# microsoft/VidTok

Hardware: NVIDIA H100
Metric: frames/sec encode+decode, kl_causal_488 17x256x256 (higher is better)
Workload: dtype bf16

## Files before the change

vidtok_b200/csrc/conv_tc.cu:

```cuda
#include <cuda.h>

#include <cstdio>
#include <cstdlib>
#include <cstring>
#include <mutex>
#include <string>
#include <type_traits>

#include "common.cuh"
#include "kernels.h"
#include "tc_host.h"
#include "tc_ptx.cuh"

namespace vt {

namespace {

thread_local std::string g_tc_err;

struct TcParams {
  int B, To, Ho, Wo, Co, Ti;
  int BW, BH, BT;
  int tilesW, tilesH, tilesT;
  int num_n_tiles, BN;
// ... 2 lines not shown
  int st, pt, ph, pw, to_off;
  int sp;
  int t_mode, cacheT;
  int stages;
  const float* bias;
  int res_mode;
  const bf16* res;
  long long rsB, rsT, rsH, rsW;
  int resT, res_t_mode, res_pool_off;
  const bf16* res_cache;
  float ra, rb;
  void* out;
  long long osB, osT, osH, osW, osC;
  int out_f32;
  int Co_real;
  int w_batched;
  int ln_mode, ln_silu;
  const float* ln_gamma;
  const float* ln_beta;
  void* out2;
  int res_mma;
  int halo, hP, a_stages;
  uint32_t halo_bytes;
  int split, a_lo, b_lo, o_lo;
  float acc_scale;
  int kparts;
  int reg_mode, reg_zc, reg_sample;
  const float* reg_noise;
  float* reg_z;
  int* reg_idx;
  double* reg_kl;
  FsqConst reg_fsq;
  uint32_t misc_off;
};

struct TcMaps {
  CUtensorMap a[4];
  CUtensorMap c;
  CUtensorMap b;
  CUtensorMap r;
  CUtensorMap e;
};

constexpr int kConsumerWarps = 8;
constexpr int kProducerWarp = kConsumerWarps;
constexpr int kThreads = (kConsumerWarps + 4) * 32;
constexpr int kABytes = 128 * 128;
constexpr uint32_t kBarTurn = 3, kBarBias = 5;

__host__ __device__ constexpr bool ping_pong(int BN, bool split) { return !split && (BN == 64 || BN == 128); }

using namespace tcx;

struct TileCoord {
  int b, t0, h0, w0, n0;
};
__device__ __forceinline__ TileCoord decode_tile(const TcParams& p, long long tile) {
  TileCoord c;
  const int nt = (int)(tile % p.num_n_tiles);
  long long m = tile / p.num_n_tiles;
  const int tw = (int)(m % p.tilesW); m /= p.tilesW;
  const int th = (int)(m % p.tilesH); m /= p.tilesH;
  const int tt = (int)(m % p.tilesT);
  c.b = (int)(m / p.tilesT);
  c.t0 = tt * p.BT; c.h0 = th * p.BH; c.w0 = tw * p.BW; c.n0 = nt * p.BN;
  return c;
}
__device__ __forceinline__ bool tap_time(const TcParams& p, const TileCoord& tc, int a, int& tv, bool& from_cache) {
  tv = (tc.t0 + p.to_off) * p.st + a - p.pt;
  from_cache = false;
  if (tv + p.BT <= 0) {
    if (p.t_mode == 0) return false;
    if (p.t_mode == 1) { tv = 0; return true; }
    from_cache = true;
    tv = p.cacheT + tv;
    return true;
  }
  return true;
}
__device__ __forceinline__ int tile_taps(const TcParams& p, const TileCoord& tc) {
  int n = 0;
  for (int a = 0; a < p.kt; ++a) {
    int tv;
    bool from_cache;
    if (tap_time(p, tc, a, tv, from_cache)) ++n;
  }
  return n;
}

__device__ __forceinline__ float quad_sum(float v) {
  v += __shfl_xor_sync(0xffffffffu, v, 1);
  v += __shfl_xor_sync(0xffffffffu, v, 2);
  return v;
}

template <int BN, bool kSplit>
__global__ void __launch_bounds__(kThreads, 1)
conv_tc_kernel(const __grid_constant__ TcMaps maps, const TcParams p) {
  extern __shared__ uint8_t smem_raw[];
  const uint32_t smem_base = (smem_u32(smem_raw) + 1023u) & ~1023u;
  uint8_t* smem_gen = smem_raw + (smem_base - smem_u32(smem_raw));
  const int warp = threadIdx.x >> 5, lane = threadIdx.x & 31;
  const uint32_t a_bytes = kABytes;
  constexpr uint32_t b_bytes = (uint32_t)BN * 128u;
  constexpr uint32_t kPl = kSplit ? 2u : 1u;
  const uint32_t stage_bytes = kPl * (p.halo ? b_bytes : a_bytes + b_bytes);
  const uint32_t win_bytes = kPl * p.halo_bytes;
  const uint32_t ring_base = smem_base + (p.halo ? (uint32_t)p.a_stages * win_bytes : 0u);
  const uint32_t bar_base = ring_base + p.stages * stage_bytes;
  auto full_bar = [&](int s) { return bar_base + 8u * s; };
  auto empty_bar = [&](int s) { return bar_base + 8u * (p.stages + s); };
  auto fullA_bar = [&](int s) { return bar_base + 8u * (2 * p.stages + s); };
  auto emptyA_bar = [&](int s) { return bar_base + 8u * (2 * p.stages + p.a_stages + s); };
  constexpr bool kPingPong = ping_pong(BN, kSplit);
  float* sbias = reinterpret_cast<float*>(smem_gen + p.misc_off);
  float* rowbuf = sbias + 2 * 768;

  if (threadIdx.x == 0) {
    constexpr uint32_t readers = kPingPong ? kConsumerWarps / 2 : kConsumerWarps;
    for (int s = 0; s < p.stages; ++s) {
      mbar_init(full_bar(s), 1);
      mbar_init(empty_bar(s), readers);
    }
    for (int s = 0; s < p.a_stages; ++s) {
      mbar_init(fullA_bar(s), 1);
      mbar_init(emptyA_bar(s), readers);
    }
    asm volatile("fence.mbarrier_init.release.cluster;" ::: "memory");
  }
  __syncthreads();

  const int nsp = p.kh * p.kw;
  const int num_kc = p.num_kc, nstages = p.stages;
  const bool halo = p.halo != 0;
  const int res_steps = p.res_mma ? BN / 64 : 0;

  if (warp >= kProducerWarp) {
    asm volatile("setmaxnreg.dec.sync.aligned.u32 40;" ::: "memory");
    if (warp != kProducerWarp) return;
    const bool el = elect_one();
    if (el) {
      prefetch_tmap(&maps.a[0]);
// ... 366 lines not shown
                  constexpr int zc = decltype(ZC)::value;
                  const long long zb = (long long)tc.b * zc * plane + pos;
#pragma unroll
                  for (int c = 0; c < zc; ++c) {
                    float zv;
                    part += kl_sample_one(f[c], f[zc + c], p.reg_sample ? p.reg_noise[zb + c * plane] : 0.f, p.reg_sample, zv);
                    p.reg_z[zb + c * plane] = zv;
                  }
                };
                if (ok) {
                  if (p.reg_zc == 4) kl_row(std::integral_constant<int, 4>());
                  else if (p.reg_zc == 8) kl_row(std::integral_constant<int, 8>());
                  else kl_row(std::integral_constant<int, 16>());
                }
                double dsum = (double)part;
#pragma unroll
                for (int o = 16; o > 0; o >>= 1) dsum += __shfl_xor_sync(0xffffffffu, dsum, o);
                if (lane == 0) atomicAdd(p.reg_kl, dsum);
              } else if (ok) {
                const long long zb = (long long)tc.b * p.reg_zc * plane + pos;
                float idx = 0.f;
#pragma unroll
                for (int c = 0; c < VT_MAX_FSQ; ++c)
                  if (c < p.reg_zc) p.reg_z[zb + c * plane] = fsq_code(p.reg_fsq, c, f[c], idx);
                if (p.reg_idx) p.reg_idx[(long long)tc.b * plane + pos] = (int)idx;
              }
            }
            asm volatile("bar.sync 2, %0;" ::"n"(kConsumerWarps * 32) : "memory");
          }
        }
        continue;
      }

      auto put = [&](void* optr, int r, int c, float y0, float y1) {
        bf16* o = reinterpret_cast<bf16*>(optr) + ooff[r] + tc.n0 + c;
        if constexpr (kSplit) {
          const uint32_t hw = pack_f16x2(y0, y1);
          *reinterpret_cast<uint32_t*>(o) = hw;
          *reinterpret_cast<uint32_t*>(o + p.o_lo) = pack_f16x2(y0 - f16_lo(hw), y1 - f16_hi(hw));
        } else {
          *reinterpret_cast<uint32_t*>(o) = pack_bf16x2(y0, y1);
        }
      };
      if constexpr (kSplit) {
        if (store_a) {
#pragma unroll
          for (int r = 0; r < 2; ++r)
            if (valid[r])
#pragma unroll
              for (int j = 0; j < BN / 8; ++j) put(p.out, r, 8 * j + cq, acc_h[4 * j + 2 * r], acc_h[4 * j + 2 * r + 1]);
        }
        if (p.ln_mode) {
          void* nout = p.ln_mode == 1 ? p.out : p.out2;
#pragma unroll
          for (int r = 0; r < 2; ++r) {
            float s = 0.f;
#pragma unroll
            for (int j = 0; j < BN / 8; ++j) s += acc_h[4 * j + 2 * r] + acc_h[4 * j + 2 * r + 1];
            const float mean = quad_sum(s) * inv_n;
            float q = 0.f;
#pragma unroll
            for (int j = 0; j < BN / 8; ++j) {
              const float d0 = acc_h[4 * j + 2 * r] - mean, d1 = acc_h[4 * j + 2 * r + 1] - mean;
              q = fmaf(d0, d0, q);
              q = fmaf(d1, d1, q);
            }
// ... 17 lines not shown
          for (int j = 0; j < BN / 8; ++j) {
            const float f0 = acc_h[4 * j + 2 * r], f1 = acc_h[4 * j + 2 * r + 1];
            s += f0 + f1;
            q = fmaf(f0, f0, q);
            q = fmaf(f1, f1, q);
            const uint32_t kp = pack_bf16x2(f0, f1);
            if (store_a && valid[r]) *reinterpret_cast<uint32_t*>(reinterpret_cast<bf16*>(p.out) + ooff[r] + tc.n0 + 8 * j + cq) = kp;
            acc_h[4 * j + 2 * r] = bf16_lo(kp);
            acc_h[4 * j + 2 * r + 1] = bf16_hi(kp);
          }
          if (!p.ln_mode) continue;
          const float mean = quad_sum(s) * inv_n;
          float var = fmaf(-mean, mean, quad_sum(q) * inv_n);
          var = var < 0.f ? 0.f : var;
          const float rstd = rsqrtf(var + 1e-6f);
          const float nmr = -mean * rstd;
          if (!valid[r]) continue;
          void* nout = p.ln_mode == 1 ? p.out : p.out2;
#pragma unroll
          for (int j = 0; j < BN / 8; ++j) {
            const int c = 8 * j + cq;
            float y0 = fmaf(fmaf(acc_h[4 * j + 2 * r], rstd, nmr), gamma_s[c], beta_s[c]);
            float y1 = fmaf(fmaf(acc_h[4 * j + 2 * r + 1], rstd, nmr), gamma_s[c + 1], beta_s[c + 1]);
            if (p.ln_silu) {
              y0 = fmaf(y0, tanh_approx(y0), y0);
              y1 = fmaf(y1, tanh_approx(y1), y1);
            }
            put(nout, r, c, y0, y1);
          }
        }
      }
    }
  }
}

__global__ void fill_identity_kernel(bf16* e, int f16, float value) {
  const int r = blockIdx.x, c = threadIdx.x;
  if (f16) reinterpret_cast<__half*>(e)[r * 256 + c] = __float2half_rn(r == c ? value : 0.0f);
  else e[r * 256 + c] = __float2bfloat16_rn(r == c ? value : 0.0f);
}

bool choose_tile(const ConvP& p, int rows, int& BW, int& BH, int& BT) {
  const bool allow_bt = (p.st == 1) && (p.t_mode == 0);
  long long best = -1;
  auto ceil_to = [](int v, int b) { return (long long)((v + b - 1) / b) * b; };
  for (int bw = 128; bw >= 8; bw >>= 1) {
    for (int bh = rows / bw; bh >= 1; bh >>= 1) {
      if (bh > 256) continue;
      const int bt = rows / (bw * bh);
      if (bt > 1 && !allow_bt) continue;
      if (bt > 16) continue;
      const long long padded = ceil_to(p.Wo, bw) * ceil_to(p.Ho, bh) * ceil_to(p.To, bt);
      const long long cost = padded * 1024 + (long long)(bw > 16 ? bw - 16 : 16 - bw) * 4 + (bt - 1);
      if (best < 0 || cost < best) { best = cost; BW = bw; BH = bh; BT = bt; }
    }
  }
  return best >= 0;
}
int choose_bn(int Co) {
  for (int bn = 256; bn >= 32; bn >>= 1)
    if (Co % bn == 0) return bn;
  return 0;
}

}

// ... 32 lines not shown
  }
  if (reg && reg->mode) {
    const int need = reg->mode == 1 ? 2 * reg->zc : reg->zc;
    const bool zc_ok = reg->mode == 1 ? (reg->zc == 4 || reg->zc == 8 || reg->zc == 16) : reg->zc <= VT_MAX_FSQ;
    if (tout == DT_F32 && Co_pad == 32 && need <= p.Co && zc_ok && p.osW == 1) t.reg = *reg;
    else g_tc_err = "regularizer epilogue needs an fp32 [B,C,T,H,W] head with Cout <= 32 holding all latent channels";
  }
  auto plan = [&](bool allow_halo, int bn_cap) -> int {
    t.halo = 0; t.hP = 0; t.a_stages = 0; t.halo_bytes = 0;
    t.BN = choose_bn(Co_pad);
    if (bn_cap && t.BN > bn_cap) t.BN = bn_cap;
    if (!choose_tile(p, 128, t.BW, t.BH, t.BT)) { g_tc_err = "no tile shape"; return -1; }
    const bool geom = p.sh == 1 && p.sw == 1 && p.kh * p.kw > 1 && p.kh <= 3 && p.kw <= 3 && p.Ho == p.Hi && p.Wo == p.Wi &&
                      w_batches <= 1 && p.Wo % 8 == 0 && p.Ho % 16 == 0;
    if (allow_halo && geom) {
      t.halo = 1;
      t.BW = 8; t.BH = 16; t.BT = 1;
      t.hP = 16;
      t.halo_bytes = (uint32_t)((16 + p.kh - 1) * t.hP * 128);
      t.a_stages = 2;
    }
    const size_t stage_bytes = (size_t)cw * ((t.halo ? 0 : (size_t)kABytes) + (size_t)t.BN * 128);
    const size_t budget = 225 * 1024;
    const size_t a_ring = (size_t)t.a_stages * t.halo_bytes * cw;
    const size_t misc = (ping_pong(t.BN, split) ? 4 : 2) * 768 * 4 + (t.reg.mode ? 128 * 33 * 4 : 0);
    const size_t fixed = 1024  + misc + 16;
    if (budget < fixed + a_ring + 2 * (stage_bytes + 16)) return 1;
    int stages = (int)((budget - fixed - a_ring) / (stage_bytes + 16));
    if (stages > 8) stages = 8;
    static const int cap = [] { const char* e = getenv("VT_TC_STAGES"); return e ? atoi(e) : 0; }();
    if (cap >= 2 && stages > cap) stages = cap;
    t.stages = stages;
    const size_t bars = 8 * (2 * (size_t)stages + 2 * (size_t)t.a_stages);
    t.misc_off = (uint32_t)((a_ring + stages * stage_bytes + bars + 15) & ~(size_t)15);
    t.smem = 1024 + t.misc_off + misc;
    t.kparts = (split && t.BN <= 128 && nk >= 16) ? (nk >= 64 ? 8 : 4) : 1;
    return 0;
  };
  const bool need_row = t.ln.mode != 0;
  const int bn_pref = (split && !need_row && w_batches <= 1) ? (nk >= 128 ? 64 : (nk >= 16 ? 128 : 0)) : 0;
  int rc = plan(true, bn_pref);
  if (rc == 1) rc = plan(false, bn_pref);
  if (rc == 1 && !need_row) rc = plan(false, 128);
  if (rc == 1) return no("not enough shared memory for 2 stages");
  if (rc != 0) return false;
  bool ident_ok = true;
  if (split) {
    const float ws = p.acc_scale != 0.f ? 1.0f / p.acc_scale : 1.0f;
    t.ident_s = ilogbf(ws);
    ident_ok = t.ident_s >= 0 && t.ident_s <= 15 && ldexpf(1.0f, t.ident_s) == ws;
  }
  t.res_mma = (ident_ok && p.res_mode == 1 && p.ra == 1.0f && p.rb == 1.0f && t.BN % 64 == 0 && p.Co % 64 == 0 && p.rsW % 8 == 0 &&
               p.rsH % 8 == 0 && p.rsT % 8 == 0 && p.rsB % 8 == 0 && (((uintptr_t)p.res) & 15) == 0) ? 1 : 0;
  *out = t;
  return true;
}

cudaError_t launch_conv_tc(const TcPlan& pl, const bf16* x, const bf16* w_nk, void* out, cudaStream_t s, long long w_batch_stride) {
  if (!tmap_encoder()) { g_tc_err = "cuTensorMapEncodeTiled unavailable"; return cudaErrorNotSupported; }
  const ConvP& p = pl.p;
  const TcRegFusion& reg = pl.reg;
  const bool split = p.split != 0;
  const int cw = split ? 2 : 1;
  if (reg.mode ? (!reg.z || (reg.mode == 1 && (!reg.kl_acc || (reg.sample && !reg.noise)))) : !out) { g_tc_err = "null output"; return cudaErrorInvalidValue; }
  if (p.t_mode == 2 && (!p.cache || p.cacheT <= 0)) { g_tc_err = "cache mode without cache"; return cudaErrorInvalidValue; }
  int dev = 0;
  const cudaError_t dev_err = current_device(dev);
  if (dev_err != cudaSuccess) { g_tc_err = "no current device, or its index is out of range"; return dev_err; }
  const int Co_pad = (p.Co + 31) / 32 * 32, Kpad = p.kt * p.kh * p.kw * p.Ci;
  TcParams t;
  memset(&t, 0, sizeof(t));
  t.BW = pl.BW; t.BH = pl.BH; t.BT = pl.BT; t.BN = pl.BN;
  t.halo = pl.halo; t.hP = pl.hP; t.a_stages = pl.a_stages; t.halo_bytes = pl.halo_bytes;
  t.stages = pl.stages; t.misc_off = pl.misc_off; t.kparts = pl.kparts; t.res_mma = pl.res_mma;
  t.tilesW = (p.Wo + t.BW - 1) / t.BW; t.tilesH = (p.Ho + t.BH - 1) / t.BH; t.tilesT = (p.To + t.BT - 1) / t.BT;
  t.num_n_tiles = Co_pad / t.BN;
  t.num_tiles = (long long)p.B * t.tilesT * t.tilesH * t.tilesW * t.num_n_tiles;
  t.split = split ? 1 : 0; t.a_lo = p.Ci; t.b_lo = Kpad; t.o_lo = p.Co;
  t.acc_scale = (split && p.acc_scale != 0.f) ? p.acc_scale : 1.0f;
  t.B = p.B; t.To = p.To; t.Ho = p.Ho; t.Wo = p.Wo; t.Co = p.Co; t.Ti = p.Ti;
  t.kt = p.kt; t.kh = p.kh; t.kw = p.kw; t.Ci = p.Ci; t.num_kc = p.Ci / 64;
  t.st = p.st; t.pt = p.pt; t.ph = p.ph; t.pw = p.pw; t.to_off = p.to_off; t.sp = p.sh;
  t.t_mode = p.t_mode; t.cacheT = p.cacheT;
  t.bias = p.bias; t.res_mode = p.res_mode; t.res = (const bf16*)p.res;
  t.rsB = p.rsB; t.rsT = p.rsT; t.rsH = p.rsH; t.rsW = p.rsW; t.resT = p.resT; t.res_t_mode = p.res_t_mode; t.res_pool_off = p.res_pool_off;
  t.res_cache = (const bf16*)p.res_cache; t.ra = p.ra; t.rb = p.rb;
  t.out = out; t.osB = p.osB; t.osT = p.osT; t.osH = p.osH; t.osW = p.osW; t.osC = p.osC;
  t.out_f32 = (pl.tout == DT_F32) ? 1 : 0;
  t.Co_real = p.Co;
  t.ln_mode = pl.ln.mode; t.ln_silu = pl.ln.silu ? 1 : 0; t.ln_gamma = pl.ln.gamma; t.ln_beta = pl.ln.beta; t.out2 = pl.ln.out2;
  if (reg.mode) {
    t.reg_mode = reg.mode; t.reg_zc = reg.zc; t.reg_sample = reg.sample; t.reg_noise = reg.noise; t.reg_z = reg.z;
    t.reg_idx = reg.indices; t.reg_kl = reg.kl_acc;
    if (reg.mode == 2) t.reg_fsq = make_fsq_const(reg.zc, reg.fsq_levels);
  }
  t.w_batched = pl.w_batches > 1 ? 1 : 0;

  TcMaps maps;
  auto encode_act = [&](CUtensorMap* m, const bf16* base, int Wn, int Hn, long long sw_, long long sh_, int Tn, long long st_, long long bs) -> bool {
    cuuint64_t dims[5] = {(cuuint64_t)(cw * p.Ci), (cuuint64_t)Wn, (cuuint64_t)Hn, (cuuint64_t)Tn, (cuuint64_t)p.B};
    cuuint64_t strides[4] = {(cuuint64_t)sw_ * 2, (cuuint64_t)sh_ * 2, (cuuint64_t)st_ * 2, (cuuint64_t)bs * 2};
    cuuint32_t box[5] = {64, (cuuint32_t)t.BW, (cuuint32_t)t.BH, (cuuint32_t)t.BT, 1};
    if (t.halo) { box[1] = (cuuint32_t)t.hP; box[2] = (cuuint32_t)(16 + p.kh - 1); }
    return encode_tmap_16b(m, 5, base, dims, strides, box, "activation", g_tc_err);
  };
  if (p.sh == 1) {
    if (!encode_act(&maps.a[0], x, p.Wi, p.Hi, p.isW, p.isH, p.Ti, p.isT, p.isB)) return cudaErrorInvalidValue;
// ... 17 lines not shown
    cuuint32_t box[3] = {64, (cuuint32_t)t.BN, 1};
    if (!encode_tmap_16b(&maps.b, 3, w_nk, dims, strides, box, "weights", g_tc_err)) return cudaErrorInvalidValue;
  }
  auto encode_out = [&](CUtensorMap* m, const void* base, int Tn, long long sW, long long sH, long long sT, long long sB, int bw, int bh, int bt) -> bool {
    cuuint64_t dims[5] = {(cuuint64_t)(cw * p.Co), (cuuint64_t)p.Wo, (cuuint64_t)p.Ho, (cuuint64_t)Tn, (cuuint64_t)p.B};
    cuuint64_t strides[4] = {(cuuint64_t)sW * 2, (cuuint64_t)sH * 2, (cuuint64_t)sT * 2, (cuuint64_t)sB * 2};
    cuuint32_t box[5] = {64, (cuuint32_t)bw, (cuuint32_t)bh, (cuuint32_t)bt, 1};
    return encode_tmap_16b(m, 5, base, dims, strides, box, "output/residual", g_tc_err);
  };
  maps.r = maps.a[0]; maps.e = maps.b;
  if (t.res_mma) {
    static bf16* ident_dev[2][kMaxDevices] = {{nullptr}};
    static std::mutex ident_mu;
    const int ik = split ? 1 : 0;
    {
      std::lock_guard<std::mutex> lock(ident_mu);
      if (!ident_dev[ik][dev]) {
        const int nmat = split ? 16 : 1;
        bf16* e = nullptr;
        cudaError_t err = cudaMalloc(&e, (size_t)nmat * 256 * 256 * sizeof(bf16));
        if (err != cudaSuccess) { g_tc_err = "cudaMalloc(identity)"; return err; }
        for (int i = 0; i < nmat; ++i) fill_identity_kernel<<<256, 256, 0, s>>>(e + (size_t)i * 256 * 256, ik, ldexpf(1.0f, i));
        if ((err = cudaStreamSynchronize(s)) != cudaSuccess) { cudaFree(e); g_tc_err = "identity fill"; return err; }
        ident_dev[ik][dev] = e;
      }
    }
    const bf16* ident = ident_dev[ik][dev] + (size_t)pl.ident_s * 256 * 256;
    if (!encode_out(&maps.r, p.res, p.resT, p.rsW, p.rsH, p.rsT, p.rsB, t.halo ? t.hP : t.BW, t.halo ? 16 + p.kh - 1 : t.BH, t.BT)) return cudaErrorInvalidValue;
    cuuint64_t dims[3] = {256, 256, 1};
    cuuint64_t strides[2] = {512, 256 * 512};
    cuuint32_t box[3] = {64, (cuuint32_t)t.BN, 1};
    if (!encode_tmap_16b(&maps.e, 3, ident, dims, strides, box, "identity", g_tc_err)) return cudaErrorInvalidValue;
  }
  {
    static SmemLimitOnce smem_limit;
    cudaError_t e = smem_limit.ensure(dev, 227 * 1024, conv_tc_kernel<32, false>, conv_tc_kernel<64, false>, conv_tc_kernel<128, false>,
                                      conv_tc_kernel<256, false>, conv_tc_kernel<32, true>, conv_tc_kernel<64, true>,
                                      conv_tc_kernel<128, true>, conv_tc_kernel<256, true>);
    if (e != cudaSuccess) { g_tc_err = "cudaFuncSetAttribute(smem)"; return e; }
  }
  const int num_sms = device_sms(dev);
  const unsigned grid = (unsigned)(t.num_tiles < num_sms ? t.num_tiles : num_sms);
  const double Mrows = (double)p.B * p.To * p.Ho * p.Wo;
  char det[160] = "";
  if (prof_enabled()) snprintf(det, sizeof(det), "k%d%d%d s%d%d %d->%d @%dx%dx%d tile%dx%dx%d bn%d%s ln%d r%d%s p%d t%d st%d", p.kt, p.kh, p.kw, p.st, p.sh, p.Ci, p.Co, p.To, p.Ho, p.Wo, t.BT, t.BH, t.BW, t.BN, t.halo ? " halo" : "", t.ln_mode, p.res_mode, t.res_mma ? "m" : "", split ? t.kparts : 1, p.t_mode, t.stages);
  ProfScope _ps(split ? "conv_tc3" : "conv_tc", 2.0 * Mrows * p.kt * p.kh * p.kw * p.Ci * p.Co,
                2.0 * cw * ((double)p.B * p.Ti * p.Hi * p.Wi * p.Ci) + Mrows * p.Co * (pl.tout == DT_F32 ? 4.0 : 2.0 * cw), s, det);
  auto launch = [&](auto kern) { kern<<<grid, kThreads, pl.smem, s>>>(maps, t); };
  switch (t.BN * 2 + (split ? 1 : 0)) {
    case 64: launch(conv_tc_kernel<32, false>); break;
    case 65: launch(conv_tc_kernel<32, true>); break;
    case 128: launch(conv_tc_kernel<64, false>); break;
    case 129: launch(conv_tc_kernel<64, true>); break;
    case 256: launch(conv_tc_kernel<128, false>); break;
    case 257: launch(conv_tc_kernel<128, true>); break;
    case 512: launch(conv_tc_kernel<256, false>); break;
    default: launch(conv_tc_kernel<256, true>); break;
  }
  count_launch();
  return cudaGetLastError();
}

}
```

vidtok_b200/csrc/kernels.h:

```cpp
#pragma once
#include <cuda_runtime.h>
#include <stdint.h>

#include "common.cuh"

namespace vt {

enum DType { DT_F32 = 0, DT_BF16 = 1, DT_SPLIT = 2 };
inline size_t dtype_size(DType t) { return t == DT_BF16 ? 2 : 4; }

void prof_start();
void prof_set_detail(bool on);
int prof_stop(char* buf, int cap);

cudaError_t launch_conv_simt(const ConvP& p, DType tin, DType tout, DType tres, const void* x, const float* w_kn,
                             void* out, cudaStream_t s);
cudaError_t launch_gemm_simt(DType ta, DType tb, DType tc, const void* A, const void* B, void* C, int M, int N, int K,
                             long long lda, long long sbn, long long sbk, long long ldc, int batch, long long bsA,
                             long long bsB, long long bsC, float scale, cudaStream_t s);

cudaError_t launch_layernorm(DType t, const void* x, const float* gamma, const float* beta, void* y, long long rows,
                             int C, bool silu, bool exact, cudaStream_t s);
cudaError_t launch_groupnorm(DType t, const void* x, const float* gamma, const float* beta, void* y, long long frames,
                             long long pos_per_frame, int C, bool per_position, bool silu, bool exact, float* stats,
// ... 46 lines not shown
cudaError_t launch_copy_frames(DType t, const void* src, void* dst, int B, long long src_bs, long long dst_bs,
                               long long n_per_batch, cudaStream_t s);

cudaError_t launch_u8_frames_to_clip(const uint8_t* src, float* dst, int T, int Hs, int Ws, int C, int h0, int w0, int H, int W,
                                    cudaStream_t s);
cudaError_t launch_clip_to_u8_frames(const float* src, uint8_t* dst, int C, int T, int H, int W, cudaStream_t s);
bool u8_frames_resize_fits(int Hs, int Ws, int C, int Hr, int Wr, int h0, int w0, int H, int W);
cudaError_t launch_u8_frames_resize_to_clip(const uint8_t* src, float* dst, int N, int Hs, int Ws, int C, int Hr, int Wr, int h0,
                                            int w0, int H, int W, int Tc, cudaStream_t s);
cudaError_t launch_split_to_f32(const bf16* x, float* y, long long rows, int C, cudaStream_t s);
cudaError_t launch_f32_to_split(const float* x, bf16* y, long long rows, int C, cudaStream_t s);

struct TcLnFusion {
  int mode = 0;
  bool silu = true;
  const float* gamma = nullptr;
  const float* beta = nullptr;
  void* out2 = nullptr;
};
struct TcRegFusion {
  int mode = 0;
  int zc = 0;
  int sample = 1;
  const float* noise = nullptr;
  float* z = nullptr;
  int* indices = nullptr;
  double* kl_acc = nullptr;
  int fsq_levels[VT_MAX_FSQ] = {0};
};
struct TcPlan {
  ConvP p;
  DType tout;
  int w_batches, BN, BW, BH, BT, halo, hP, a_stages, stages, kparts, res_mma, ident_s;
  uint32_t halo_bytes, misc_off;
  size_t smem;
  TcLnFusion ln;
  TcRegFusion reg;
};
bool conv_tc_plan(const ConvP& p, DType tout, const TcLnFusion* ln, const TcRegFusion* reg, int w_batches, TcPlan* out);
cudaError_t launch_conv_tc(const TcPlan& pl, const bf16* x, const bf16* w_nk, void* out, cudaStream_t s, long long w_batch_stride = 0);
cudaError_t launch_kl_clear(double* scratch, cudaStream_t s);
cudaError_t launch_kl_finish(const double* scratch, int B, float* kl_loss, cudaStream_t s);
cudaError_t launch_tap_planes_gather(const bf16* P, const float* bias, float* out, int B, int Ti, int H, int W, int NP, int Co,
                                     int to_off, cudaStream_t s, int pt = 2);
cudaError_t launch_pack_w_tap_planes(const float* w, bf16* out, int Co, int Ci, int NP, cudaStream_t s);
cudaError_t launch_transpose_bf16(const bf16* x, bf16* y, int batch, int rows, int cols, cudaStream_t s, bool split = false);
const char* conv_tc_last_error();

bool tblock_tc_supported(int B, int T, int H, int W, int C);
struct TbCache {
  const bf16* n1_in = nullptr;
  const bf16* h_in = nullptr;
  bf16* n1_out = nullptr;
  bf16* h_out = nullptr;
};
cudaError_t launch_tblock_tc(const bf16* n1, const bf16* x, const bf16* w1, const float* bias1, const float* gamma2,
                             const float* beta2, const bf16* w2, const float* bias2, bf16* out, bf16* out2,
                             const float* gamma_out, const float* beta_out, bool out_silu, int B, int T, int H, int W,
                             cudaStream_t s, const TbCache* cache = nullptr);
const char* tblock_tc_last_error();

bool attn_tc_supported(long long frames, long long tokens, int C, bool split);
size_t attn_tc_workspace(long long frames, long long tokens, int C, bool split);
cudaError_t launch_attn_tc(const bf16* q, const bf16* k, const bf16* v, bf16* o, int frames, int H, int W, int C, bool split,
                           void* ws, cudaStream_t s);
const char* attn_tc_last_error();
// ... 7 lines not shown
```

vidtok_b200/csrc/tblock_tc.cu:

```cuda
#include <cuda.h>

#include <cstdio>
#include <cstring>
#include <string>

#include "common.cuh"
#include "kernels.h"
#include "tc_host.h"
#include "tc_ptx.cuh"

namespace vt {

namespace {
using namespace tcx;

thread_local std::string g_tb_err;
constexpr int kC = 128;
constexpr int kKc = kC / 64;
constexpr uint32_t kTile = 128 * 128;
constexpr int kHSlots = 3;
constexpr int kConsumerWarps = 8;
constexpr int kProducerWarp = kConsumerWarps;
constexpr int kThreadsTb = (kConsumerWarps + 4) * 32;

// ... 119 lines not shown
    pend_stage = -1;
  };
  auto kstep = [&](bool a_from_stage, uint32_t h_addr, uint32_t scale) {
    mbar_wait(full_bar(stage), phase);
    const uint32_t sa = ring_base + stage * stage_bytes;
    const uint32_t al = desc_lo(a_from_stage ? sa + (uint32_t)g * 64u * 128u : h_addr), bl = desc_lo(sa + kTile);
    wgmma_fence();
#pragma unroll
    for (uint32_t j = 0; j < 4u; ++j) wgmma_k16<kC, false>(acc, desc(al + 2u * j, hi), desc(bl + 2u * j, hi), j == 0 ? scale : 1u);
    wgmma_commit();
    wgmma_wait<1>();
    release();
    pend_stage = stage;
    if (++stage == p.stages) { stage = 0; phase ^= 1u; }
  };
  auto finish = [&]() {
    wgmma_wait<0>();
    acc_fence(acc);
    release();
  };
  auto wg_sync = [&]() { asm volatile("bar.sync %0, 128;" ::"r"(1 + g) : "memory"); };
  const float* bias1 = cst;
  const float* g2 = cst + kC;
  const float* b2 = cst + 2 * kC;
  const float* bias2 = cst + 3 * kC;
  const float* g3 = cst + 4 * kC;
  const float* b3 = cst + 5 * kC;
  const int cq = 2 * (lane & 3);
  const int rbase = 64 * g + 16 * wq + (lane >> 2);
  const bool front = kCache && p.cached_in;
  const int gtid = threadIdx.x & 127;
  auto slot_of = [&](int tv) { return h_base + (uint32_t)((tv + kHSlots) % kHSlots) * kKc * kTile; };
  auto ring_unit = [&](uint32_t slot, int row, int c) {
    return reinterpret_cast<uint4*>(smem_gen + (slot - smem_base) + (c >> 6) * kTile + row * 128 + ((((c & 63) >> 3) ^ (row & 7)) << 4));
  };

  for (long long strip = blockIdx.x; strip < p.num_strips; strip += gridDim.x) {
    const int tw = (int)(strip % p.tilesW);
    const int th = (int)((strip / p.tilesW) % p.tilesH);
    const int b = (int)(strip / ((long long)p.tilesW * p.tilesH));
    long long pos0[2];
#pragma unroll
    for (int r = 0; r < 2; ++r) {
      const int row = rbase + 8 * r;
      const int h = th * p.BH + row / p.BW, w = tw * p.BW + row % p.BW;
      pos0[r] = (((long long)b * p.T) * p.H + h) * p.W + w;
    }
    const long long frame = (long long)p.H * p.W;
    auto cache_pos = [&](int i, int j, int& row) {
      row = 64 * g + (i >> 4);
      const int h = th * p.BH + row / p.BW, w = tw * p.BW + row % p.BW;
      return ((((long long)b * 2 + j) * p.H + h) * p.W + w) * kC + (i & 15) * 8;
    };
    if (front) {
      if (gtid == 0) bulk_wait_read<0>();
      wg_sync();
      for (int j = 0; j < 2; ++j)
        for (int i = gtid; i < 64 * 16; i += 128) {
          int row;
          const long long off = cache_pos(i, j, row);
          *ring_unit(slot_of(j - 2), row, (i & 15) * 8) = *reinterpret_cast<const uint4*>(p.ch_in + off);
        }
      fence_async_smem();
      wg_sync();
    }
    const int box_w = tw * p.BW + (64 * g) % p.BW, box_h = th * p.BH + (64 * g) / p.BW;
    auto x_load = [&](int t) {
// ... 2 lines not shown
      mbar_expect_tx(x_bar(g), (uint32_t)kKc * 64u * 128u);
      for (int kc = 0; kc < kKc; ++kc) tma_load_5d(dst + (uint32_t)kc * kTile, &maps.x, x_bar(g), kc * 64, box_w, box_h, t, b);
    };
    for (int t = 0; t < p.T; ++t) {
      uint32_t scale = 0;
      for (int a = 0; a < 3; ++a) {
        if (t - 2 + a < 0 && !front) continue;
        for (int kc = 0; kc < kKc; ++kc) { kstep(true, 0u, scale); scale = 1; }
      }
      finish();
      if (gtid == 0) bulk_wait_read<0>();
      wg_sync();
      const uint32_t slot = h_base + (uint32_t)(t % kHSlots) * kKc * kTile;
#pragma unroll
      for (int r = 0; r < 2; ++r) {
        float s = 0.f, q = 0.f;
#pragma unroll
        for (int j = 0; j < kC / 8; ++j) {
          const int c = 8 * j + cq;
          const float f0 = acc[4 * j + 2 * r] + bias1[c], f1 = acc[4 * j + 2 * r + 1] + bias1[c + 1];
          s += f0 + f1;
          q = fmaf(f0, f0, q);
          q = fmaf(f1, f1, q);
          const uint32_t kp = pack_bf16x2(f0, f1);
          acc[4 * j + 2 * r] = bf16_lo(kp);
          acc[4 * j + 2 * r + 1] = bf16_hi(kp);
        }
        const float mean = quad_sum(s) * (1.0f / kC);
        float var = fmaf(-mean, mean, quad_sum(q) * (1.0f / kC));
        var = var < 0.f ? 0.f : var;
        const float rstd = rsqrtf(var + 1e-6f);
        const float nmr = -mean * rstd;
        const int row = rbase + 8 * r;
        uint8_t* hrow = smem_gen + (slot - smem_base) + row * 128;
#pragma unroll
        for (int j = 0; j < kC / 8; ++j) {
          const int c = 8 * j + cq;
          float y0 = fmaf(fmaf(acc[4 * j + 2 * r], rstd, nmr), g2[c], b2[c]);
          float y1 = fmaf(fmaf(acc[4 * j + 2 * r + 1], rstd, nmr), g2[c + 1], b2[c + 1]);
          y0 = fmaf(y0, tanh_approx(y0), y0);
          y1 = fmaf(y1, tanh_approx(y1), y1);
          const int cc = c & 63, u = cc >> 3;
          *reinterpret_cast<uint32_t*>(hrow + (c >> 6) * kTile + ((u ^ (row & 7)) << 4) + (cc & 7) * 2) = pack_bf16x2(y0, y1);
        }
      }
      fence_async_smem();
      wg_sync();
      const bool tap0 = t >= 2 || front;
      if (!tap0) x_load(t);
      scale = 0;
      int s2 = 0;
      for (int a = 0; a < 3; ++a) {
        const int tv = t - 2 + a;
        if (tv < 0 && !front) continue;
        const uint32_t hs = (kCache ? slot_of(tv) : h_base + (uint32_t)(tv % kHSlots) * kKc * kTile) + (uint32_t)g * 64u * 128u;
        for (int kc = 0; kc < kKc; ++kc) {
          kstep(false, hs + (uint32_t)kc * kTile, scale);
          scale = 1;
          if (++s2 == kKc + 1 && tap0) { wg_sync(); x_load(t); }
        }
      }
      finish();
      mbar_wait(x_bar(g), xphase);
      xphase ^= 1u;
      const uint32_t xslot = slot_of(t - 2);
#pragma unroll
      for (int r = 0; r < 2; ++r) {
        const long long off = (pos0[r] + (long long)t * frame) * kC;
        const int row = rbase + 8 * r;
        uint8_t* xrow = smem_gen + (xslot - smem_base) + row * 128;
        float s = 0.f, q = 0.f;
#pragma unroll
        for (int j = 0; j < kC / 8; ++j) {
          const int c = 8 * j + cq;
          const int cc = c & 63, u = cc >> 3;
          uint32_t* xo = reinterpret_cast<uint32_t*>(xrow + (c >> 6) * kTile + ((u ^ (row & 7)) << 4) + (cc & 7) * 2);
          const uint32_t xw = *xo;
          const float f0 = acc[4 * j + 2 * r] + bias2[c] + bf16_lo(xw), f1 = acc[4 * j + 2 * r + 1] + bias2[c + 1] + bf16_hi(xw);
          s += f0 + f1;
          q = fmaf(f0, f0, q);
          q = fmaf(f1, f1, q);
          const uint32_t kp = pack_bf16x2(f0, f1);
          *xo = kp;
          acc[4 * j + 2 * r] = bf16_lo(kp);
          acc[4 * j + 2 * r + 1] = bf16_hi(kp);
        }
        if (!p.ln_out) continue;
        const float mean = quad_sum(s) * (1.0f / kC);
        float var = fmaf(-mean, mean, quad_sum(q) * (1.0f / kC));
        var = var < 0.f ? 0.f : var;
        const float rstd = rsqrtf(var + 1e-6f);
        const float nmr = -mean * rstd;
        bf16* o2 = p.out2 + off;
#pragma unroll
        for (int j = 0; j < kC / 8; ++j) {
          const int c = 8 * j + cq;
          float y0 = fmaf(fmaf(acc[4 * j + 2 * r], rstd, nmr), g3[c], b3[c]);
          float y1 = fmaf(fmaf(acc[4 * j + 2 * r + 1], rstd, nmr), g3[c + 1], b3[c + 1]);
          if (p.ln_out_silu) {
            y0 = fmaf(y0, tanh_approx(y0), y0);
            y1 = fmaf(y1, tanh_approx(y1), y1);
          }
          *reinterpret_cast<uint32_t*>(o2 + c) = pack_bf16x2(y0, y1);
        }
      }
      fence_async_smem();
      wg_sync();
      if (gtid == 0) {
        for (int kc = 0; kc < kKc; ++kc)
// ... 121 lines not shown
```

vidtok_b200/csrc/tc_ptx.cuh:

```cuda
#pragma once
#include <cuda.h>
#include <cuda_bf16.h>
#include <cuda_fp16.h>
#include <stdint.h>

namespace vt {
namespace tcx {
__device__ __forceinline__ uint32_t smem_u32(const void* p) { return (uint32_t)__cvta_generic_to_shared(p); }

__device__ __forceinline__ void mbar_init(uint32_t bar, uint32_t count) {
  asm volatile("mbarrier.init.shared::cta.b64 [%0], %1;" ::"r"(bar), "r"(count) : "memory");
}
__device__ __forceinline__ void mbar_expect_tx(uint32_t bar, uint32_t bytes) {
  asm volatile("mbarrier.arrive.expect_tx.shared::cta.b64 _, [%0], %1;" ::"r"(bar), "r"(bytes) : "memory");
}
__device__ __forceinline__ void mbar_arrive(uint32_t bar) {
  asm volatile("mbarrier.arrive.shared::cta.b64 _, [%0];" ::"r"(bar) : "memory");
}
__device__ __forceinline__ bool mbar_try_wait(uint32_t bar, uint32_t parity) {
  uint32_t ok;
  asm volatile(
      "{\n\t"
      ".reg .pred p;\n\t"
      "mbarrier.try_wait.parity.shared::cta.b64 p, [%1], %2;\n\t"
// ... 39 lines not shown
  asm volatile("bar.sync %0, %1;" ::"r"(id), "r"(threads) : "memory");
}
__device__ __forceinline__ void named_bar_arrive(uint32_t id, uint32_t threads) {
  asm volatile("bar.arrive %0, %1;" ::"r"(id), "r"(threads) : "memory");
}
__device__ __forceinline__ void prefetch_tmap(const CUtensorMap* map) {
  asm volatile("prefetch.tensormap [%0];" ::"l"(map) : "memory");
}
__device__ __forceinline__ bool elect_one() {
  uint32_t pred;
  asm volatile(
      "{\n\t"
      ".reg .pred P1;\n\t"
      "elect.sync _|P1, 0xffffffff;\n\t"
      "selp.u32 %0, 1, 0, P1;\n\t"
      "}"
      : "=r"(pred));
  return pred != 0;
}

__device__ __forceinline__ void wgmma_fence() { asm volatile("wgmma.fence.sync.aligned;" ::: "memory"); }
__device__ __forceinline__ void wgmma_commit() { asm volatile("wgmma.commit_group.sync.aligned;" ::: "memory"); }
template <int kPending>
__device__ __forceinline__ void wgmma_wait() { asm volatile("wgmma.wait_group.sync.aligned %0;" ::"n"(kPending) : "memory"); }
template <int R>
__device__ __forceinline__ void acc_fence(float (&d)[R]) {
#pragma unroll
  for (int i = 0; i < R; ++i) asm volatile("" : "+f"(d[i])::"memory");
}

__device__ __forceinline__ uint32_t desc_lo(uint32_t saddr) { return ((saddr & 0x3FFFFu) >> 4) | (1u << 16); }
__device__ __forceinline__ uint32_t desc_hi(uint32_t sbo) { return (sbo >> 4) | (1u << 30); }
__device__ __forceinline__ uint64_t desc(uint32_t lo, uint32_t hi) { return ((uint64_t)hi << 32) | lo; }

__device__ __forceinline__ void wgmma_32_bf16(float (&d)[16], uint64_t da, uint64_t db, uint32_t scale_d) {
  asm volatile(
      "{\n\t.reg .pred p;\n\t"
      "setp.ne.b32 p, %18, 0;\n\t"
      "wgmma.mma_async.sync.aligned.m64n32k16.f32.bf16.bf16 "
      "{"
      "%0, %1, %2, %3, %4, %5, %6, %7, %8, %9, %10, %11, %12, %13, %14, %15"
      "}, %16, %17, p, 1, 1, 0, 0;\n\t}"
      : "+f"(d[0]), "+f"(d[1]), "+f"(d[2]), "+f"(d[3]), "+f"(d[4]), "+f"(d[5]), "+f"(d[6]), "+f"(d[7]),
        "+f"(d[8]), "+f"(d[9]), "+f"(d[10]), "+f"(d[11]), "+f"(d[12]), "+f"(d[13]), "+f"(d[14]), "+f"(d[15])
      : "l"(da), "l"(db), "r"(scale_d));
}
__device__ __forceinline__ void wgmma_32_f16(float (&d)[16], uint64_t da, uint64_t db, uint32_t scale_d) {
  asm volatile(
      "{\n\t.reg .pred p;\n\t"
      "setp.ne.b32 p, %18, 0;\n\t"
      "wgmma.mma_async.sync.aligned.m64n32k16.f32.f16.f16 "
      "{"
      "%0, %1, %2, %3, %4, %5, %6, %7, %8, %9, %10, %11, %12, %13, %14, %15"
      "}, %16, %17, p, 1, 1, 0, 0;\n\t}"
      : "+f"(d[0]), "+f"(d[1]), "+f"(d[2]), "+f"(d[3]), "+f"(d[4]), "+f"(d[5]), "+f"(d[6]), "+f"(d[7]),
        "+f"(d[8]), "+f"(d[9]), "+f"(d[10]), "+f"(d[11]), "+f"(d[12]), "+f"(d[13]), "+f"(d[14]), "+f"(d[15])
      : "l"(da), "l"(db), "r"(scale_d));
}
__device__ __forceinline__ void wgmma_64_bf16(float (&d)[32], uint64_t da, uint64_t db, uint32_t scale_d) {
  asm volatile(
      "{\n\t.reg .pred p;\n\t"
      "setp.ne.b32 p, %34, 0;\n\t"
      "wgmma.mma_async.sync.aligned.m64n64k16.f32.bf16.bf16 "
      "{"
      "%0, %1, %2, %3, %4, %5, %6, %7, %8, %9, %10, %11, %12, %13, %14, %15, "
      "%16, %17, %18, %19, %20, %21, %22, %23, %24, %25, %26, %27, %28, %29, %30, %31"
// ... 177 lines not shown
```

Measured before the change: 460.9.

## Stage BN=256 bf16 conv epilogue outputs through swizzled smem and TMA stores

Adds a staged-output variant of the tensor-core conv kernel for non-split bf16 BN=256 tiles. The epilogue writes bf16 results, including the fused LayerNorm/SiLU output, into a 128B-swizzled shared buffer and issues 5D TMA bulk stores per 64-channel chunk instead of scattered per-thread global stores. Each consumer half uses its own named barrier and waits on bulk reads before reusing its buffer. This costs extra shared memory and synchronisation, and is only enabled when the smem budget and 16-byte output alignment allow. The swizzle address math in the tblock kernel is also pulled into a shared helper.

```diff
diff --git a/vidtok_b200/csrc/conv_tc.cu b/vidtok_b200/csrc/conv_tc.cu
--- a/vidtok_b200/csrc/conv_tc.cu
+++ b/vidtok_b200/csrc/conv_tc.cu
@@ -58,6 +58,10 @@
   double* reg_kl;
   FsqConst reg_fsq;
   uint32_t misc_off;
+  int stage_out;
+  uint32_t stage_smem;
+  uint32_t stage_off;
+  int half_dim, half_ext;
 };
 
 struct TcMaps {
@@ -66,13 +70,15 @@
   CUtensorMap b;
   CUtensorMap r;
   CUtensorMap e;
+  CUtensorMap o, o2;
 };
 
 constexpr int kConsumerWarps = 8;
 constexpr int kProducerWarp = kConsumerWarps;
 constexpr int kThreads = (kConsumerWarps + 4) * 32;
 constexpr int kABytes = 128 * 128;
-constexpr uint32_t kBarTurn = 3, kBarBias = 5;
+constexpr uint32_t kBarTurn = 3, kBarBias = 5, kBarStage = 7;
+constexpr uint32_t kStageOutBytes = 64 * 128;
 
 __host__ __device__ constexpr bool ping_pong(int BN, bool split) { return !split && (BN == 64 || BN == 128); }
 
@@ -120,7 +126,7 @@
   return v;
 }
 
-template <int BN, bool kSplit>
+template <int BN, bool kSplit, bool kStage = false>
 __global__ void __launch_bounds__(kThreads, 1)
 conv_tc_kernel(const __grid_constant__ TcMaps maps, const TcParams p) {
   extern __shared__ uint8_t smem_raw[];
@@ -133,7 +139,7 @@
   const uint32_t stage_bytes = kPl * (p.halo ? b_bytes : a_bytes + b_bytes);
   const uint32_t win_bytes = kPl * p.halo_bytes;
   const uint32_t ring_base = smem_base + (p.halo ? (uint32_t)p.a_stages * win_bytes : 0u);
-  const uint32_t bar_base = ring_base + p.stages * stage_bytes;
+  const uint32_t bar_base = ring_base + p.stages * stage_bytes + p.stage_smem;
   auto full_bar = [&](int s) { return bar_base + 8u * s; };
   auto empty_bar = [&](int s) { return bar_base + 8u * (p.stages + s); };
   auto fullA_bar = [&](int s) { return bar_base + 8u * (2 * p.stages + s); };
@@ -566,6 +572,85 @@
         continue;
       }
 
+      if constexpr (kStage) {
+        static_assert(!kSplit && BN == 256, "staged stores: the cooperative bf16 schedule");
+        {
+          float rstd[2], nmr[2];
+#pragma unroll
+          for (int r = 0; r < 2; ++r) {
+            float s = 0.f, q = 0.f;
+#pragma unroll
+            for (int j = 0; j < BN / 8; ++j) {
+              const float f0 = acc_h[4 * j + 2 * r], f1 = acc_h[4 * j + 2 * r + 1];
+              s += f0 + f1;
+              q = fmaf(f0, f0, q);
+              q = fmaf(f1, f1, q);
+              const uint32_t kp = pack_bf16x2(f0, f1);
+              acc_h[4 * j + 2 * r] = bf16_lo(kp);
+              acc_h[4 * j + 2 * r + 1] = bf16_hi(kp);
+            }
+            const float mean = quad_sum(s) * inv_n;
+            float var = fmaf(-mean, mean, quad_sum(q) * inv_n);
+            var = var < 0.f ? 0.f : var;
+            rstd[r] = rsqrtf(var + 1e-6f);
+            nmr[r] = -mean * rstd[r];
+          }
+          const uint32_t sbuf = smem_base + p.stage_off + (uint32_t)(row0 >> 6) * kStageOutBytes;
+          const uint32_t sw = sbuf + swz128_unit(row0 & 63, 0) + 2u * cq;
+          auto put_s = [&](int r, int u, uint32_t word) {
+            asm volatile("st.shared.b32 [%0], %1;" ::"r"((sw ^ ((uint32_t)u << 4)) + 1024u * r), "r"(word) : "memory");
+          };
+          const bool issuer = (threadIdx.x & 127) == 0;
+          auto reserve = [&]() {
+            if (issuer) bulk_wait_read<0>();
+            named_bar_sync(kBarStage + g, 128);
+          };
+          auto send = [&](const CUtensorMap* m, int k) {
+            fence_async_smem();
+            named_bar_sync(kBarStage + g, 128);
+            if (issuer) {
+              const int ho = g * p.half_ext;
+              tma_store_5d(m, sbuf, tc.n0 + 64 * k, tc.w0 + (p.half_dim == 1 ? ho : 0), tc.h0 + (p.half_dim == 2 ? ho : 0),
+                           tc.t0 + (p.half_dim == 3 ? ho : 0), tc.b);
+              bulk_commit();
+            }
+          };
+          if (store_a) {
+#pragma unroll
+            for (int k = 0; k < BN / 64; ++k) {
+              reserve();
+#pragma unroll
+              for (int r = 0; r < 2; ++r)
+#pragma unroll
+                for (int u = 0; u < 8; ++u) put_s(r, u, pack_bf16x2(acc_h[4 * (8 * k + u) + 2 * r], acc_h[4 * (8 * k + u) + 2 * r + 1]));
+              send(&maps.o, k);
+            }
+          }
+          if (p.ln_mode) {
+            const CUtensorMap* nmap = p.ln_mode == 1 ? &maps.o : &maps.o2;
+#pragma unroll
+            for (int k = 0; k < BN / 64; ++k) {
+              reserve();
+#pragma unroll
+              for (int r = 0; r < 2; ++r)
+#pragma unroll
+                for (int u = 0; u < 8; ++u) {
+                  const int j = 8 * k + u, c = 8 * j + cq;
+                  float y0 = fmaf(fmaf(acc_h[4 * j + 2 * r], rstd[r], nmr[r]), gamma_s[c], beta_s[c]);
+                  float y1 = fmaf(fmaf(acc_h[4 * j + 2 * r + 1], rstd[r], nmr[r]), gamma_s[c + 1], beta_s[c + 1]);
+                  if (p.ln_silu) {
+                    y0 = fmaf(y0, tanh_approx(y0), y0);
+                    y1 = fmaf(y1, tanh_approx(y1), y1);
+                  }
+                  put_s(r, u, pack_bf16x2(y0, y1));
+                }
+              send(nmap, k);
+            }
+          }
+          continue;
+        }
+      }
+
       auto put = [&](void* optr, int r, int c, float y0, float y1) {
         bf16* o = reinterpret_cast<bf16*>(optr) + ooff[r] + tc.n0 + c;
         if constexpr (kSplit) {
@@ -649,6 +734,7 @@
       }
     }
   }
+  if (kStage && (threadIdx.x & 127) == 0) bulk_wait<0>();
 }
 
 __global__ void fill_identity_kernel(bf16* e, int f16, float value) {
@@ -747,7 +833,11 @@
     if (cap >= 2 && stages > cap) stages = cap;
     t.stages = stages;
     const size_t bars = 8 * (2 * (size_t)stages + 2 * (size_t)t.a_stages);
-    t.misc_off = (uint32_t)((a_ring + stages * stage_bytes + bars + 15) & ~(size_t)15);
+    const size_t staging = 2 * (size_t)kStageOutBytes;
+    const bool staged = !split && tout == DT_BF16 && t.BN == 256 &&
+                        1024 + ((a_ring + stages * stage_bytes + staging + bars + 15) & ~(size_t)15) + misc <= 227 * 1024;
+    t.stage_out = staged ? 1 : 0;
+    t.misc_off = (uint32_t)((a_ring + stages * stage_bytes + (staged ? staging : 0) + bars + 15) & ~(size_t)15);
     t.smem = 1024 + t.misc_off + misc;
     t.kparts = (split && t.BN <= 128 && nk >= 16) ? (nk >= 64 ? 8 : 4) : 1;
     return 0;
@@ -788,6 +878,9 @@
   t.BW = pl.BW; t.BH = pl.BH; t.BT = pl.BT; t.BN = pl.BN;
   t.halo = pl.halo; t.hP = pl.hP; t.a_stages = pl.a_stages; t.halo_bytes = pl.halo_bytes;
   t.stages = pl.stages; t.misc_off = pl.misc_off; t.kparts = pl.kparts; t.res_mma = pl.res_mma;
+  t.stage_smem = pl.stage_out ? 2 * kStageOutBytes : 0;
+  t.stage_off = (uint32_t)pl.a_stages * pl.halo_bytes + (uint32_t)pl.stages * (uint32_t)((pl.halo ? 0 : kABytes) + pl.BN * 128);
+  t.stage_out = (pl.stage_out && ((uintptr_t)out & 15) == 0 && ((uintptr_t)pl.ln.out2 & 15) == 0) ? 1 : 0;
   t.tilesW = (p.Wo + t.BW - 1) / t.BW; t.tilesH = (p.Ho + t.BH - 1) / t.BH; t.tilesT = (p.To + t.BT - 1) / t.BT;
   t.num_n_tiles = Co_pad / t.BN;
   t.num_tiles = (long long)p.B * t.tilesT * t.tilesH * t.tilesW * t.num_n_tiles;
@@ -871,11 +964,21 @@
     cuuint32_t box[3] = {64, (cuuint32_t)t.BN, 1};
     if (!encode_tmap_16b(&maps.e, 3, ident, dims, strides, box, "identity", g_tc_err)) return cudaErrorInvalidValue;
   }
+  if (t.stage_out) {
+    int hb[3] = {t.BW, t.BH, t.BT};
+    t.half_dim = t.BT > 1 ? 3 : (t.BH > 1 ? 2 : 1);
+    t.half_ext = (hb[t.half_dim - 1] /= 2);
+    if (!encode_out(&maps.o, out, p.To, p.osW, p.osH, p.osT, p.osB, hb[0], hb[1], hb[2])) return cudaErrorInvalidValue;
+    maps.o2 = maps.o;
+    if (t.ln_mode == 2 && !encode_out(&maps.o2, t.out2, p.To, p.osW, p.osH, p.osT, p.osB, hb[0], hb[1], hb[2])) return cudaErrorInvalidValue;
+  } else {
+    maps.o = maps.o2 = maps.a[0];
+  }
   {
     static SmemLimitOnce smem_limit;
     cudaError_t e = smem_limit.ensure(dev, 227 * 1024, conv_tc_kernel<32, false>, conv_tc_kernel<64, false>, conv_tc_kernel<128, false>,
                                       conv_tc_kernel<256, false>, conv_tc_kernel<32, true>, conv_tc_kernel<64, true>,
-                                      conv_tc_kernel<128, true>, conv_tc_kernel<256, true>);
+                                      conv_tc_kernel<128, true>, conv_tc_kernel<256, true>, conv_tc_kernel<256, false, true>);
     if (e != cudaSuccess) { g_tc_err = "cudaFuncSetAttribute(smem)"; return e; }
   }
   const int num_sms = device_sms(dev);
@@ -886,7 +989,8 @@
   ProfScope _ps(split ? "conv_tc3" : "conv_tc", 2.0 * Mrows * p.kt * p.kh * p.kw * p.Ci * p.Co,
                 2.0 * cw * ((double)p.B * p.Ti * p.Hi * p.Wi * p.Ci) + Mrows * p.Co * (pl.tout == DT_F32 ? 4.0 : 2.0 * cw), s, det);
   auto launch = [&](auto kern) { kern<<<grid, kThreads, pl.smem, s>>>(maps, t); };
-  switch (t.BN * 2 + (split ? 1 : 0)) {
+  if (t.stage_out) launch(conv_tc_kernel<256, false, true>);
+  else switch (t.BN * 2 + (split ? 1 : 0)) {
     case 64: launch(conv_tc_kernel<32, false>); break;
     case 65: launch(conv_tc_kernel<32, true>); break;
     case 128: launch(conv_tc_kernel<64, false>); break;
diff --git a/vidtok_b200/csrc/kernels.h b/vidtok_b200/csrc/kernels.h
--- a/vidtok_b200/csrc/kernels.h
+++ b/vidtok_b200/csrc/kernels.h
@@ -102,6 +102,7 @@
   ConvP p;
   DType tout;
   int w_batches, BN, BW, BH, BT, halo, hP, a_stages, stages, kparts, res_mma, ident_s;
+  int stage_out;
   uint32_t halo_bytes, misc_off;
   size_t smem;
   TcLnFusion ln;
diff --git a/vidtok_b200/csrc/tblock_tc.cu b/vidtok_b200/csrc/tblock_tc.cu
--- a/vidtok_b200/csrc/tblock_tc.cu
+++ b/vidtok_b200/csrc/tblock_tc.cu
@@ -175,7 +175,7 @@
   const int gtid = threadIdx.x & 127;
   auto slot_of = [&](int tv) { return h_base + (uint32_t)((tv + kHSlots) % kHSlots) * kKc * kTile; };
   auto ring_unit = [&](uint32_t slot, int row, int c) {
-    return reinterpret_cast<uint4*>(smem_gen + (slot - smem_base) + (c >> 6) * kTile + row * 128 + ((((c & 63) >> 3) ^ (row & 7)) << 4));
+    return reinterpret_cast<uint4*>(smem_gen + (slot - smem_base) + (c >> 6) * kTile + swz128_unit(row, (c & 63) >> 3));
   };
 
   for (long long strip = blockIdx.x; strip < p.num_strips; strip += gridDim.x) {
@@ -244,7 +244,7 @@
         const float rstd = rsqrtf(var + 1e-6f);
         const float nmr = -mean * rstd;
         const int row = rbase + 8 * r;
-        uint8_t* hrow = smem_gen + (slot - smem_base) + row * 128;
+        uint8_t* hslot = smem_gen + (slot - smem_base);
 #pragma unroll
         for (int j = 0; j < kC / 8; ++j) {
           const int c = 8 * j + cq;
@@ -252,8 +252,8 @@
           float y1 = fmaf(fmaf(acc[4 * j + 2 * r + 1], rstd, nmr), g2[c + 1], b2[c + 1]);
           y0 = fmaf(y0, tanh_approx(y0), y0);
           y1 = fmaf(y1, tanh_approx(y1), y1);
-          const int cc = c & 63, u = cc >> 3;
-          *reinterpret_cast<uint32_t*>(hrow + (c >> 6) * kTile + ((u ^ (row & 7)) << 4) + (cc & 7) * 2) = pack_bf16x2(y0, y1);
+          const int cc = c & 63;
+          *reinterpret_cast<uint32_t*>(hslot + (c >> 6) * kTile + swz128_unit(row, cc >> 3) + (cc & 7) * 2) = pack_bf16x2(y0, y1);
         }
       }
       fence_async_smem();
@@ -280,13 +280,13 @@
       for (int r = 0; r < 2; ++r) {
         const long long off = (pos0[r] + (long long)t * frame) * kC;
         const int row = rbase + 8 * r;
-        uint8_t* xrow = smem_gen + (xslot - smem_base) + row * 128;
+        uint8_t* xs = smem_gen + (xslot - smem_base);
         float s = 0.f, q = 0.f;
 #pragma unroll
         for (int j = 0; j < kC / 8; ++j) {
           const int c = 8 * j + cq;
-          const int cc = c & 63, u = cc >> 3;
-          uint32_t* xo = reinterpret_cast<uint32_t*>(xrow + (c >> 6) * kTile + ((u ^ (row & 7)) << 4) + (cc & 7) * 2);
+          const int cc = c & 63;
+          uint32_t* xo = reinterpret_cast<uint32_t*>(xs + (c >> 6) * kTile + swz128_unit(row, cc >> 3) + (cc & 7) * 2);
           const uint32_t xw = *xo;
           const float f0 = acc[4 * j + 2 * r] + bias2[c] + bf16_lo(xw), f1 = acc[4 * j + 2 * r + 1] + bias2[c + 1] + bf16_hi(xw);
           s += f0 + f1;
diff --git a/vidtok_b200/csrc/tc_ptx.cuh b/vidtok_b200/csrc/tc_ptx.cuh
--- a/vidtok_b200/csrc/tc_ptx.cuh
+++ b/vidtok_b200/csrc/tc_ptx.cuh
@@ -95,6 +95,7 @@
 __device__ __forceinline__ uint32_t desc_lo(uint32_t saddr) { return ((saddr & 0x3FFFFu) >> 4) | (1u << 16); }
 __device__ __forceinline__ uint32_t desc_hi(uint32_t sbo) { return (sbo >> 4) | (1u << 30); }
 __device__ __forceinline__ uint64_t desc(uint32_t lo, uint32_t hi) { return ((uint64_t)hi << 32) | lo; }
+__device__ __forceinline__ uint32_t swz128_unit(int row, int u) { return (uint32_t)row * 128u + (uint32_t)((u ^ (row & 7)) << 4); }
 
 __device__ __forceinline__ void wgmma_32_bf16(float (&d)[16], uint64_t da, uint64_t db, uint32_t scale_d) {
   asm volatile(
```

Result: faster. 475.0, median of 6 (+3.1%).
